# robot-learning-freiburg/MM-DistillNet

Measured on AMD Instinct MI355X. Metric: distillation-step images/sec (3 teachers + audio student, D2, bs=8), higher is better.
Workload: dtype f32; 1 GPU; BASELINE configs[2]: full 3-teacher (RGB+thermal+depth) -> audio student distillation step, EfficientDet-D2, 512x512, per-GPU batch 8, fwd+losses+bwd+all-reduce+Adam; global_batch=8, image_size=512, parallelism=dp1, graph=True, full=False

## Files before the change

mm_distillnet_amd/csrc/elt.hip:

```cpp
#include "common.h"
#include <cstdlib>

#define ROWS_PER_BLOCK 256
static inline int elt_rows_per_block(long long M, int C, bool reduces = false) {
  const long long blocks = (long long)cdiv(C, 64) * cdiv(M, ROWS_PER_BLOCK);
  int rpb = blocks >= 1024 ? ROWS_PER_BLOCK : (blocks >= 256 ? 128 : 64);
  while (reduces && rpb < ROWS_PER_BLOCK && cdiv(M, rpb) > 64) rpb *= 2;
  return rpb;
}

__device__ __forceinline__ float4 red_rowgroups(float4 v) {
  v.x += __shfl_xor(v.x, 16, 64); v.y += __shfl_xor(v.y, 16, 64); v.z += __shfl_xor(v.z, 16, 64); v.w += __shfl_xor(v.w, 16, 64);
  v.x += __shfl_xor(v.x, 32, 64); v.y += __shfl_xor(v.y, 32, 64); v.z += __shfl_xor(v.z, 32, 64); v.w += __shfl_xor(v.w, 32, 64);
  return v;
}
__device__ __forceinline__ float block_chan_sum(float4 v, float* sRed , int tid) {
  v = red_rowgroups(v);
  __syncthreads();
  if ((tid & 63) < 16) *reinterpret_cast<float4*>(&sRed[(tid >> 6) * 64 + (tid & 15) * 4]) = v;
  __syncthreads();
  float r = 0.f;
  if (tid < 64) r = sRed[tid] + sRed[64 + tid] + sRed[128 + tid] + sRed[192 + tid];
  return r;
}
// ... 248 lines not shown
  if (images_per_group <= 0 || w_stride <= 0 || bn_stride <= 0 || (w_stride & 3) || (bn_stride & 3)) return MMD_EINVAL;
  g_group = MmdGroup{n_groups, images_per_group, w_stride, bn_stride};
  g_group_read = false;
  return MMD_OK;
}

template <bool Q>
__global__ __launch_bounds__(256) void se_hidden_kernel(const void* __restrict__ pooled_, const float* __restrict__ wr,
                                                        const float* __restrict__ br, float* __restrict__ hpre, int C, int S,
                                                        int g_images, long long g_w) {
  const int b = blockIdx.x, wave = threadIdx.x >> 6, lane = threadIdx.x & 63;
  const int j = blockIdx.y * 4 + wave;
  if (j >= S) return;
  if (g_images) { const size_t o = (size_t)(b / g_images) * g_w; wr += o; br += o; }
  const float* p = reinterpret_cast<const float*>(pooled_) + (size_t)b * C;
  const long long* pq = reinterpret_cast<const long long*>(pooled_) + (size_t)b * C;
  const float* w = wr + (size_t)j * C;
  float acc = 0.f;
#pragma unroll 4
  for (int c = lane * 4; c < C; c += 256) {
    float4 a;
    if (Q) {
      const longlong2 q0 = *reinterpret_cast<const longlong2*>(pq + c), q1 = *reinterpret_cast<const longlong2*>(pq + c + 2);
      a = make_float4(mmd_pool_get(q0.x), mmd_pool_get(q0.y), mmd_pool_get(q1.x), mmd_pool_get(q1.y));
    } else {
      a = mmd_ld4(p + c);
    }
    const float4 q = mmd_ld4(w + c);
    acc += a.x * q.x + a.y * q.y + a.z * q.z + a.w * q.w;
  }
  acc = wave_sum(acc);
  if (lane == 0) hpre[(size_t)b * S + j] = acc + br[j];
}
__global__ __launch_bounds__(256) void se_gate_kernel(const float* __restrict__ hpre, const float* __restrict__ wet,
                                                      const float* __restrict__ be, float* __restrict__ gate, int C, int S,
                                                      int g_images, long long g_w) {
  __shared__ float sh[256];
  const int b = blockIdx.x;
  if (g_images) { const size_t o = (size_t)(b / g_images) * g_w; wet += o; be += o; }
  for (int j = threadIdx.x; j < S; j += 256) sh[j] = mmd_swish(hpre[(size_t)b * S + j]);
  __syncthreads();
  const int c = blockIdx.y * 256 + threadIdx.x;
  if (c >= C) return;
  float acc = be[c];
#pragma unroll 8
  for (int j = 0; j < S; ++j) acc += wet[(size_t)j * C + c] * sh[j];
  gate[(size_t)b * C + c] = mmd_sigmoid(acc);
}
static int se_fc_fwd_impl(const void* pooled, bool q, const float* wr, const float* br, const float* we, const float* be,
                          float* hpre, float* gate, int B, int C, int S, hipStream_t stream) {
  if (!pooled || !wr || !br || !we || !be || !hpre || !gate || B <= 0 || C <= 0 || (C & 3) || S <= 0 || S > 256) return MMD_EINVAL;
  const MmdGroup& gr = mmd_group();
  const int gi = gr.n > 1 ? gr.images : 0;
  if (gi && B != gr.n * gr.images) return MMD_EINVAL;
  mmd_prof_tag(MMD_FAM_SE, "sefwd B%lld C%lld S%lld q%lld", B, C, S, q ? 1 : 0);
  mmd_prof_begin(MMD_FAM_SE, stream);
  if (q) hipLaunchKernelGGL(se_hidden_kernel<true>, dim3(B, cdiv(S, 4)), dim3(256), 0, stream, pooled, wr, br, hpre, C, S, gi, gr.w_stride);
  else hipLaunchKernelGGL(se_hidden_kernel<false>, dim3(B, cdiv(S, 4)), dim3(256), 0, stream, pooled, wr, br, hpre, C, S, gi, gr.w_stride);
  hipLaunchKernelGGL(se_gate_kernel, dim3(B, cdiv(C, 256)), dim3(256), 0, stream, hpre, we, be, gate, C, S, gi, gr.w_stride);
  mmd_prof_end(MMD_FAM_SE, stream, 4.0 * B * (double)C * S, 4.0 * ((gr.n > 1 ? gr.n : 1) * 2.0 * C * S + (double)B * ((q ? 3.0 : 2.0) * C + 2.0 * S)));
  return mmd_check_launch();
}
extern "C" int mmd_se_fc_fwd(const float* pooled, const float* wr, const float* br, const float* we, const float* be,
                             float* hpre, float* gate, int B, int C, int S, hipStream_t stream) {
  return se_fc_fwd_impl(pooled, false, wr, br, we, be, hpre, gate, B, C, S, stream);
}
extern "C" int mmd_se_fc_fwd_q(const long long* pooled_q, const float* wr, const float* br, const float* we, const float* be,
                               float* hpre, float* gate, int B, int C, int S, hipStream_t stream) {
  return se_fc_fwd_impl(pooled_q, true, wr, br, we, be, hpre, gate, B, C, S, stream);
}

__global__ __launch_bounds__(256) void se_bwd_a_kernel(const float* __restrict__ dgate, const float* __restrict__ gate,
                                                       const float* __restrict__ wet, float* __restrict__ dpe, float* dh,
                                                       int C, int S) {
  const int b = blockIdx.x, wave = threadIdx.x >> 6, lane = threadIdx.x & 63;
  const int j = blockIdx.y * 4 + wave;
  if (j >= S) return;
  const float* gp = gate + (size_t)b * C;
  const float* dp = dgate + (size_t)b * C;
  const float* wp = wet + (size_t)j * C;
  float acc = 0.f;
#pragma unroll 4
  for (int c = lane * 4; c < C; c += 256) {
    const float4 g = mmd_ld4(gp + c), dg = mmd_ld4(dp + c), w = mmd_ld4(wp + c);
    const float4 d = make_float4(dg.x * g.x * (1.f - g.x), dg.y * g.y * (1.f - g.y), dg.z * g.z * (1.f - g.z), dg.w * g.w * (1.f - g.w));
    if (j == 0) mmd_st4(dpe + (size_t)b * C + c, d);
    acc += w.x * d.x + w.y * d.y + w.z * d.z + w.w * d.w;
  }
  acc = wave_sum(acc);
  if (lane == 0) dh[(size_t)b * S + j] = acc;
}
__global__ __launch_bounds__(256) void se_bwd_b_kernel(const float* __restrict__ dh, const float* __restrict__ hpre,
                                                       const float* __restrict__ wr, float* __restrict__ dpr,
                                                       float* __restrict__ dpooled, float dpool_scale, int C, int S,
                                                       const float* __restrict__ gate, const float* __restrict__ pool5,
                                                       double* bn_sums, int B) {
  __shared__ float sd[256];
  const int b = blockIdx.x, tid = threadIdx.x;
  for (int j = tid; j < S; j += 256) {
    float d = dh[(size_t)b * S + j] * mmd_swish_grad(hpre[(size_t)b * S + j]);
    sd[j] = d;
    if (blockIdx.y == 0) dpr[(size_t)b * S + j] = d;
  }
  __syncthreads();
  const int c = blockIdx.y * 256 + tid;
  if (c >= C) return;
  float acc = 0.f;
#pragma unroll 8
  for (int j = 0; j < S; ++j) acc += wr[(size_t)j * C + c] * sd[j];
  const float dp = acc * dpool_scale;
  dpooled[(size_t)b * C + c] = dp;
  if (bn_sums) {
    const size_t i = (size_t)b * C + c, n = (size_t)B * C;
    const float gt = gate[i];
    atomicAdd(&bn_sums[c], (double)(gt * pool5[n + i] + dp * pool5[3 * n + i]));
    atomicAdd(&bn_sums[C + c], (double)(gt * pool5[2 * n + i] + dp * pool5[4 * n + i]));
  }
}
__global__ void se_fc_wgrad_kernel(const float* __restrict__ dpe, const float* __restrict__ dpr,
                                   const float* __restrict__ hpre, const float* __restrict__ pooled, float* dwr, float* dbr,
                                   float* dwe, float* dbe, int B, int C, int S) {
  int i = blockIdx.x * blockDim.x + threadIdx.x;
  if (i >= C * S) return;
  {
    int j = i / C, c = i % C;
    float acc = 0.f, accb = 0.f;
    for (int b = 0; b < B; ++b) {
      float d = dpe[(size_t)b * C + c];
      acc += d * mmd_swish(hpre[(size_t)b * S + j]);
      accb += d;
    }
    dwe[i] += acc;
    if (j == 0) dbe[c] += accb;
  }
  {
    int j = i / C, c = i % C;
    float acc = 0.f, accb = 0.f;
    for (int b = 0; b < B; ++b) {
      float d = dpr[(size_t)b * S + j];
      acc += d * pooled[(size_t)b * C + c];
      accb += d;
    }
    dwr[i] += acc;
    if (c == 0) dbr[j] += accb;
  }
}
extern "C" int mmd_se_fc_bwd(const float* dgate, const float* gate, const float* hpre, const float* pooled,
                             const float* wr, const float* we, float* dpe_ws, float* dpr_ws, float* dh_zeroed,
                             float* dpooled, float dpool_scale, float* dwr, float* dbr, float* dwe, float* dbe, int B,
                             int C, int S, const float* pool5, double* bn_sums, hipStream_t stream) {
  if (!dgate || !gate || !hpre || !pooled || !wr || !we || !dpe_ws || !dpr_ws || !dh_zeroed || !dpooled) return MMD_EINVAL;
  if (dwr && (!dbr || !dwe || !dbe)) return MMD_EINVAL;
  if (B <= 0 || C <= 0 || (C & 3) || S <= 0 || S > 256 || ((pool5 == nullptr) != (bn_sums == nullptr))) return MMD_EINVAL;
  mmd_prof_tag(MMD_FAM_SE, "sebwd B%lld C%lld S%lld", B, C, S, 0);
  mmd_prof_begin(MMD_FAM_SE, stream);
  hipLaunchKernelGGL(se_bwd_a_kernel, dim3(B, cdiv(S, 4)), dim3(256), 0, stream, dgate, gate, we, dpe_ws, dh_zeroed, C, S);
  hipLaunchKernelGGL(se_bwd_b_kernel, dim3(B, cdiv(C, 256)), dim3(256), 0, stream, dh_zeroed, hpre, wr, dpr_ws, dpooled,
                     dpool_scale, C, S, gate, pool5, bn_sums, B);
  if (dwr)
    hipLaunchKernelGGL(se_fc_wgrad_kernel, dim3(cdiv((long long)C * S, 256)), dim3(256), 0, stream, dpe_ws, dpr_ws, hpre,
                       pooled, dwr, dbr, dwe, dbe, B, C, S);
  mmd_prof_end(MMD_FAM_SE, stream, 4.0 * B * (double)C * S, 4.0 * (2.0 * C * S + (double)B * (4.0 * C + 3.0 * S)));
  return mmd_check_launch();
}
#define SE_MAXC 3072
__global__ __launch_bounds__(256) void se_bwd_ab_kernel(const float* __restrict__ dgate, const float* __restrict__ gate,
                                                        const float* __restrict__ hpre, const float* __restrict__ wr,
                                                        const float* __restrict__ wet, float* __restrict__ dpe, float* __restrict__ dpr,
                                                        float* __restrict__ dpooled, float dpool_scale, int C, int S,
                                                        const float* __restrict__ pool5, double* bn_sums, int B) {
  __shared__ float sdpe[SE_MAXC];
  __shared__ float sd[256];
  const int b = blockIdx.x, tid = threadIdx.x, wave = tid >> 6, lane = tid & 63;
  for (int c = tid; c < C; c += 256) {
    const float g = gate[(size_t)b * C + c];
    const float d = dgate[(size_t)b * C + c] * g * (1.f - g);
    sdpe[c] = d;
    if (blockIdx.y == 0) dpe[(size_t)b * C + c] = d;
  }
  __syncthreads();
  for (int j = wave; j < S; j += 4) {
    const float* w = wet + (size_t)j * C;
    float acc = 0.f;
    for (int c = lane; c < C; c += 64) acc += w[c] * sdpe[c];
    acc = wave_sum(acc);
    if (lane == 0) {
      const float d = acc * mmd_swish_grad(hpre[(size_t)b * S + j]);
      sd[j] = d;
      if (blockIdx.y == 0) dpr[(size_t)b * S + j] = d;
    }
  }
  __syncthreads();
  const int c = blockIdx.y * 256 + tid;
  if (c >= C) return;
  float acc = 0.f;
#pragma unroll 8
  for (int j = 0; j < S; ++j) acc += wr[(size_t)j * C + c] * sd[j];
  const float dp = acc * dpool_scale;
  dpooled[(size_t)b * C + c] = dp;
  if (bn_sums) {
    const size_t i = (size_t)b * C + c, n = (size_t)B * C;
    const float gt = gate[i];
    atomicAdd(&bn_sums[c], (double)(gt * pool5[n + i] + dp * pool5[3 * n + i]));
    atomicAdd(&bn_sums[C + c], (double)(gt * pool5[2 * n + i] + dp * pool5[4 * n + i]));
  }
}
extern "C" int mmd_se_fc_bwd_fused(const float* dgate, const float* gate, const float* hpre, const float* wr, const float* we,
                                   float* dpe_ws, float* dpr_ws, float* dpooled, float dpool_scale, int B, int C, int S,
                                   const float* pool5, double* bn_sums, hipStream_t stream) {
  if (!dgate || !gate || !hpre || !wr || !we || !dpe_ws || !dpr_ws || !dpooled) return MMD_EINVAL;
  if (B <= 0 || C <= 0 || C > SE_MAXC || S <= 0 || S > 256 || ((pool5 == nullptr) != (bn_sums == nullptr))) return MMD_EINVAL;
  mmd_prof_tag(MMD_FAM_SE, "sebwdf B%lld C%lld S%lld", B, C, S, 0);
  mmd_prof_begin(MMD_FAM_SE, stream);
  hipLaunchKernelGGL(se_bwd_ab_kernel, dim3(B, cdiv(C, 256)), dim3(256), 0, stream, dgate, gate, hpre, wr, we, dpe_ws, dpr_ws, dpooled,
                     dpool_scale, C, S, pool5, bn_sums, B);
  mmd_prof_end(MMD_FAM_SE, stream, 4.0 * B * (double)C * S, 4.0 * (2.0 * C * S + (double)B * (4.0 * C + 3.0 * S)));
  return mmd_check_launch();
}

struct SeWgDesc { const float* dpe; const float* dpr; const float* hpre; const float* pooled; float* dwr; float* dbr; float* dwe; float* dbe;
                  long long C; long long S; };
__global__ void se_fc_wgrad_batched_kernel(const SeWgDesc* __restrict__ desc, int B) {
  const SeWgDesc d = desc[blockIdx.y];
  const int C = (int)d.C, S = (int)d.S;
  const int i = blockIdx.x * blockDim.x + threadIdx.x;
  if (i >= C * S) return;
  const int j = i / C, c = i % C;
  float a1 = 0.f, b1 = 0.f, a2 = 0.f, b2 = 0.f;
  for (int b = 0; b < B; ++b) {
    const float pe = mmd_ldg(d.dpe + (size_t)b * C + c), pr = mmd_ldg(d.dpr + (size_t)b * S + j);
    a1 += pe * mmd_swish(mmd_ldg(d.hpre + (size_t)b * S + j)); b1 += pe;
    a2 += pr * mmd_ldg(d.pooled + (size_t)b * C + c); b2 += pr;
  }
  mmd_stg(d.dwe + i, mmd_ldg(d.dwe + i) + a1);
  if (j == 0) mmd_stg(d.dbe + c, mmd_ldg(d.dbe + c) + b1);
  mmd_stg(d.dwr + i, mmd_ldg(d.dwr + i) + a2);
  if (c == 0) mmd_stg(d.dbr + j, mmd_ldg(d.dbr + j) + b2);
}
extern "C" int mmd_se_fc_wgrad_batched(const void* desc, int n, int max_cs, int B, hipStream_t stream) {
  if (!desc || n <= 0 || max_cs <= 0 || B <= 0) return MMD_EINVAL;
  hipLaunchKernelGGL(se_fc_wgrad_batched_kernel, dim3(cdiv(max_cs, 256), n), dim3(256), 0, stream, (const SeWgDesc*)desc, B);
  return mmd_check_launch();
}

extern "C" int mmd_se_fc_wgrad(const float* dpe, const float* dpr, const float* hpre, const float* pooled, float* dwr, float* dbr,
                               float* dwe, float* dbe, int B, int C, int S, hipStream_t stream) {
  if (!dpe || !dpr || !hpre || !pooled || !dwr || !dbr || !dwe || !dbe || B <= 0 || C <= 0 || S <= 0 || S > 256) return MMD_EINVAL;
  hipLaunchKernelGGL(se_fc_wgrad_kernel, dim3(cdiv((long long)C * S, 256)), dim3(256), 0, stream, dpe, dpr, hpre, pooled, dwr,
// ... 495 lines not shown
```

mm_distillnet_amd/csrc/mbconv_fused.hip:

```cpp
#include "common.h"
#include <cstdlib>

struct MbxArgs {
  const float* x; const float* w0; const float* sc0; const float* sh0;
  const float* wd; const float* sc1; const float* sh1;
  float* y; long long* pool; float pool_scale;
  int B, H, W, Cin, C, OH, OW, pad_t, pad_l, tiles_h, tiles_w, cchunks;
  int y16;
  int g_images; long long g_w, g_bn;
};

template <int K, int S> struct MbxCfg;
template <> struct MbxCfg<3, 1> { static constexpr int TH = 16, TW = 16, R = 4; };
template <> struct MbxCfg<5, 1> { static constexpr int TH = 16, TW = 16, R = 4; };
template <> struct MbxCfg<3, 2> { static constexpr int TH = 8, TW = 8, R = 1; };
template <> struct MbxCfg<5, 2> { static constexpr int TH = 8, TW = 8, R = 1; };

constexpr int MBX_CC = 48;
constexpr int MBX_LD = 20;
constexpr int MBX_NW = 4;
static_assert(MBX_NW == 4, "the pool epilogue adds four wave slots in a fixed order");

template <int CTRL> __device__ __forceinline__ float mbx_dpp(float v) {
  return __int_as_float(__builtin_amdgcn_update_dpp(0, __float_as_int(v), CTRL, 0xf, 0xf, false));
}

template <int NK, int K, int S>
__global__ __launch_bounds__(MBX_NW * 64) void mbx_kernel(MbxArgs a) {
  using Cf = MbxCfg<K, S>;
  constexpr int TH = Cf::TH, TW = Cf::TW, R = Cf::R, NW = MBX_NW;
  constexpr int IH = (TH - 1) * S + K, IW = (TW - 1) * S + K, P = IH * IW;
  constexpr int PT = (P + 15) / 16, TPW = (PT + NW - 1) / NW;
  constexpr int NT = NW * 64, NG = NT / 4, CC = MBX_CC, LD = MBX_LD;
  constexpr int SEG = (R - 1) * S + K, NSTRIP = TH * (TW / R);
  constexpr int W0S = 4 * NK + 4;
  extern __shared__ float smem[];
  float* const sE = smem;
  float* const sW = smem + PT * 16 * LD;
  float* const sPool = sW + K * K * CC;
  float* const sAff = sPool + NW * CC;
  float* const sW0 = sAff + 4 * CC;
  const int tid = threadIdx.x, lane = tid & 63, r = lane & 15, g = lane >> 4;
  const int wave = __builtin_amdgcn_readfirstlane(tid >> 6);
  int bid = mmd_xcd_swizzle(blockIdx.x, gridDim.x);
  const int cc = bid % a.cchunks; bid /= a.cchunks;
  const int tw = bid % a.tiles_w; bid /= a.tiles_w;
  const int th = bid % a.tiles_h; bid /= a.tiles_h;
  const int b = bid, c0 = cc * CC;
  if (a.g_images) {
    const size_t gw = (size_t)(b / a.g_images) * a.g_w, gb = (size_t)(b / a.g_images) * a.g_bn;
    a.w0 += gw; a.wd += gw; a.sc0 += gb; a.sh0 += gb; a.sc1 += gb; a.sh1 += gb;
  }
  const int oh0 = th * TH, ow0 = tw * TW, ih0 = oh0 * S - a.pad_t, iw0 = ow0 * S - a.pad_l;
  const int H = a.H, W = a.W, Cin = a.Cin;

  float bx[TPW][NK];
  bool in[TPW];
  {
    const float* xb = a.x + (size_t)b * H * W * Cin + g * NK;
#pragma unroll
    for (int t = 0; t < TPW; ++t) {
      const int p = (wave + t * NW) * 16 + r;
      const int pr = p / IW, pc = p - pr * IW;
      const int ih = ih0 + pr, iw = iw0 + pc;
      in[t] = p < P && ih >= 0 && ih < H && iw >= 0 && iw < W;
      const int ihc = min(max(ih, 0), H - 1), iwc = min(max(iw, 0), W - 1);
      const float* xp = xb + ((size_t)ihc * W + iwc) * Cin;
      if (NK % 4 == 0) {
#pragma unroll
        for (int j = 0; j < NK; j += 4) {
          const float4 v = mmd_ld4(xp + j);
          bx[t][j] = v.x; bx[t][j + 1] = v.y; bx[t][j + 2] = v.z; bx[t][j + 3] = v.w;
        }
      } else {
#pragma unroll
      for (int j = 0; j < NK; j += 2) {
        const float2 v = *reinterpret_cast<const float2*>(xp + j);
        bx[t][j] = v.x; bx[t][j + 1] = v.y;
      }
      }
    }
  }
  for (int i = tid; i < K * K * 12; i += NT) {
    const int tap = i / 12, q = (i % 12) * 4;
    *reinterpret_cast<float4*>(&sW[tap * CC + q]) = mmd_ld4(a.wd + (size_t)tap * a.C + c0 + q);
  }
  for (int i = tid; i < CC * NK; i += NT) {
    const int n = i / NK, k4 = i - n * NK;
    *reinterpret_cast<float4*>(&sW0[n * W0S + k4 * 4]) = mmd_ld4(a.w0 + (size_t)c0 * Cin + i * 4);
  }
  if (tid < CC) {
    sAff[tid] = a.sc0[c0 + tid]; sAff[CC + tid] = a.sh0[c0 + tid]; sAff[2 * CC + tid] = a.sc1[c0 + tid]; sAff[3 * CC + tid] = a.sh1[c0 + tid];
  }
  __syncthreads();

  constexpr unsigned SPERM = S == 1 ? 0x73261540u : 0x76452310u;
  const int qd = tid & 3, grp = ((tid >> 5) << 3) + (int)((SPERM >> (((tid >> 2) & 7) * 4)) & 7u), c4 = qd * 4;
#pragma unroll 1
  for (int ct = 0; ct < 3; ++ct) {
    {
      float aw[NK];
      const float* wp = sW0 + (ct * 16 + r) * W0S + g * NK;
#pragma unroll
      for (int j = 0; j < NK; j += 2) {
        const float2 v = *reinterpret_cast<const float2*>(wp + j);
        aw[j] = v.x; aw[j + 1] = v.y;
      }
      const float4 s0 = *reinterpret_cast<const float4*>(&sAff[ct * 16 + 4 * g]), h0 = *reinterpret_cast<const float4*>(&sAff[CC + ct * 16 + 4 * g]);
#pragma unroll
      for (int t = 0; t < TPW; ++t) {
        const int tile = wave + t * NW;
        if (tile >= PT) break;
        f32x4 acc = f32x4{0.f, 0.f, 0.f, 0.f};
#pragma unroll
        for (int j = 0; j < NK; ++j) acc = __builtin_amdgcn_mfma_f32_16x16x4f32(aw[j], bx[t][j], acc, 0, 0, 0);
        float4 v;
        v.x = mmd_swish(acc[0] * s0.x + h0.x); v.y = mmd_swish(acc[1] * s0.y + h0.y);
        v.z = mmd_swish(acc[2] * s0.z + h0.z); v.w = mmd_swish(acc[3] * s0.w + h0.w);
        if (!in[t]) v = make_float4(0.f, 0.f, 0.f, 0.f);
        *reinterpret_cast<float4*>(&sE[(tile * 16 + r) * LD + 4 * g]) = v;
      }
    }
    __syncthreads();

    float4 pl = make_float4(0.f, 0.f, 0.f, 0.f);
    {
      const int cb = c0 + ct * 16 + c4;
      const float4 osc = *reinterpret_cast<const float4*>(&sAff[2 * CC + ct * 16 + c4]), osh = *reinterpret_cast<const float4*>(&sAff[3 * CC + ct * 16 + c4]);
      const float* const sWc = sW + ct * 16 + c4;
      for (int s = grp; s < NSTRIP; s += NG) {
        const int orow = s / (TW / R), ocol0 = (s % (TW / R)) * R;
        float4 acc[R];
#pragma unroll
        for (int o = 0; o < R; ++o) acc[o] = make_float4(0.f, 0.f, 0.f, 0.f);
#pragma unroll(K == 3 ? 3 : 1)
        for (int i = 0; i < K; ++i) {
          float4 in4[SEG];
          const float* prow = &sE[((orow * S + i) * IW + ocol0 * S) * LD + c4];
#pragma unroll
          for (int q = 0; q < SEG; ++q) in4[q] = *reinterpret_cast<const float4*>(prow + q * LD);
#pragma unroll
          for (int j = 0; j < K; ++j) {
            const float4 wv = *reinterpret_cast<const float4*>(&sWc[(i * K + j) * CC]);
#pragma unroll
            for (int o = 0; o < R; ++o) {
              acc[o].x += in4[o * S + j].x * wv.x; acc[o].y += in4[o * S + j].y * wv.y;
              acc[o].z += in4[o * S + j].z * wv.z; acc[o].w += in4[o * S + j].w * wv.w;
            }
          }
        }
        const int oh = oh0 + orow;
#pragma unroll
        for (int o = 0; o < R; ++o) {
          const int ow = ow0 + ocol0 + o;
          if (oh < a.OH && ow < a.OW) {
            float4 t;
            t.x = mmd_swish(acc[o].x * osc.x + osh.x); t.y = mmd_swish(acc[o].y * osc.y + osh.y);
            t.z = mmd_swish(acc[o].z * osc.z + osh.z); t.w = mmd_swish(acc[o].w * osc.w + osh.w);
            pl.x += t.x; pl.y += t.y; pl.z += t.z; pl.w += t.w;
            mmd_stw4(a.y, (((size_t)b * a.OH + oh) * a.OW + ow) * a.C + cb, t, a.y16);
          }
        }
      }
    }
    if (a.pool) {
      pl.x += mbx_dpp<0x124>(pl.x); pl.y += mbx_dpp<0x124>(pl.y); pl.z += mbx_dpp<0x124>(pl.z); pl.w += mbx_dpp<0x124>(pl.w);
      pl.x += mbx_dpp<0x128>(pl.x); pl.y += mbx_dpp<0x128>(pl.y); pl.z += mbx_dpp<0x128>(pl.z); pl.w += mbx_dpp<0x128>(pl.w);
      pl.x += __shfl_xor(pl.x, 16, 64); pl.y += __shfl_xor(pl.y, 16, 64); pl.z += __shfl_xor(pl.z, 16, 64); pl.w += __shfl_xor(pl.w, 16, 64);
      pl.x += __shfl_xor(pl.x, 32, 64); pl.y += __shfl_xor(pl.y, 32, 64); pl.z += __shfl_xor(pl.z, 32, 64); pl.w += __shfl_xor(pl.w, 32, 64);
      if (lane < 4) *reinterpret_cast<float4*>(sPool + wave * CC + ct * 16 + c4) = pl;
    }
    __syncthreads();
  }
  if (a.pool && tid < CC)
    mmd_pool_add(&a.pool[(size_t)b * a.C + c0 + tid], ((sPool[tid] + sPool[CC + tid]) + sPool[2 * CC + tid]) + sPool[3 * CC + tid], a.pool_scale);
}

static int mbx_same_pad_lo(int n, int k, int s, int* out) {
  int o = (n + s - 1) / s;
  int extra = (o - 1) * s - n + k;
  if (extra < 0) extra = 0;
  *out = o;
  return extra / 2;
}

template <int NK, int K, int S>
static int mbx_launch(MbxArgs& a, hipStream_t st) {
  using Cf = MbxCfg<K, S>;
  a.tiles_h = cdiv(a.OH, Cf::TH); a.tiles_w = cdiv(a.OW, Cf::TW); a.cchunks = a.C / MBX_CC;
  const long long nb = (long long)a.B * a.tiles_h * a.tiles_w * a.cchunks;
  if (nb > 0x7fffffffLL) return MMD_EINVAL;
  constexpr int IH = (Cf::TH - 1) * S + K, IW = (Cf::TW - 1) * S + K;
  constexpr size_t lds = (size_t)((IH * IW + 15) / 16 * 16 * MBX_LD + K * K * MBX_CC + (4 + MBX_NW) * MBX_CC + MBX_CC * (4 * NK + 4)) * sizeof(float);
  static_assert(lds <= 64 * 1024, "tile does not fit the default dynamic LDS limit");
  hipLaunchKernelGGL((mbx_kernel<NK, K, S>), dim3((unsigned)nb), dim3(MBX_NW * 64), lds, st, a);
  return mmd_check_launch();
}

template <int NK>
static int mbx_launch_ks(MbxArgs& a, int k, int s, hipStream_t st) {
  if (k == 3 && s == 1) return mbx_launch<NK, 3, 1>(a, st);
  if (k == 3 && s == 2) return mbx_launch<NK, 3, 2>(a, st);
  if (k == 5 && s == 1) return mbx_launch<NK, 5, 1>(a, st);
  return mbx_launch<NK, 5, 2>(a, st);
}

extern "C" int mmd_mbconv_expand_dw_supported(int Cin, int Cmid, int k, int stride) {
  if ((k != 3 && k != 5) || (stride != 1 && stride != 2)) return 0;
  if (Cmid <= 0 || Cmid % MBX_CC) return 0;
  return Cin == 16 || Cin == 24 || Cin == 32 || Cin == 40 || Cin == 48 || Cin == 56;
}

static int mbx_impl(const float* x, const float* w_expand, const float* scale0, const float* shift0,
                    const float* w_dw, const float* scale1, const float* shift1, float* y, long long* pool,
                    int B, int H, int W, int Cin, int Cmid, int k, int stride, int y16, hipStream_t stream) {
  if (!x || !w_expand || !scale0 || !shift0 || !w_dw || !scale1 || !shift1 || !y || B <= 0 || H <= 0 || W <= 0) return MMD_EINVAL;
  if (!mmd_mbconv_expand_dw_supported(Cin, Cmid, k, stride)) return MMD_EINVAL;
  MbxArgs a{};
  a.x = x; a.w0 = w_expand; a.sc0 = scale0; a.sh0 = shift0; a.wd = w_dw; a.sc1 = scale1; a.sh1 = shift1; a.y = y; a.pool = pool;
  a.B = B; a.H = H; a.W = W; a.Cin = Cin; a.C = Cmid;
  a.pad_t = mbx_same_pad_lo(H, k, stride, &a.OH); a.pad_l = mbx_same_pad_lo(W, k, stride, &a.OW);
  a.pool_scale = 1.0f / (float)((long long)a.OH * a.OW);
  a.y16 = y16;
  if (mmd_group_on()) {
    const MmdGroup& gr = mmd_group();
    if (B != gr.n * gr.images || y16) return MMD_EINVAL;
    a.g_images = gr.images; a.g_w = gr.w_stride; a.g_bn = gr.bn_stride;
// ... 28 lines not shown
```

Measured before the change: 597.0 images/sec.

## Fuse SE forward FCs into one kernel and prefetch gate-weight columns

Adds a single-launch SE forward kernel that stages pooled activations in shared memory, computes the hidden FC with multi-row wave dot products, and then computes the gate FC in the same block. This removes a launch and the round trip of the hidden activations through global memory. The column dot products now prefetch the first 32 weight rows into registers before the barrier, and the fused backward kernel is reused for the unfused bwd path when no weight grads are needed. The cost is redundant hidden-FC work per C-tile block, which is limited by a byte threshold, plus higher register pressure.

```diff
diff --git a/mm_distillnet_amd/csrc/elt.hip b/mm_distillnet_amd/csrc/elt.hip
--- a/mm_distillnet_amd/csrc/elt.hip
+++ b/mm_distillnet_amd/csrc/elt.hip
@@ -304,20 +304,117 @@
   acc = wave_sum(acc);
   if (lane == 0) hpre[(size_t)b * S + j] = acc + br[j];
 }
+#define SE_GU 32
+struct SeCol { float v[SE_GU]; };
+__device__ __forceinline__ SeCol se_col_load(const float* __restrict__ w, int C, int c, int S, int j0) {
+  SeCol q;
+#pragma unroll
+  for (int u = 0; u < SE_GU; ++u) q.v[u] = w[(size_t)min(j0 + u, S - 1) * C + c];
+  return q;
+}
+__device__ __forceinline__ float se_col_add(float acc, const SeCol& q, const float* sh, int S, int j0) {
+  if (j0 + SE_GU <= S) {
+#pragma unroll
+    for (int u = 0; u < SE_GU; ++u) acc += q.v[u] * sh[j0 + u];
+  } else {
+#pragma unroll
+    for (int u = 0; u < SE_GU; ++u)
+      if (j0 + u < S) acc += q.v[u] * sh[j0 + u];
+  }
+  return acc;
+}
+__device__ __forceinline__ float se_col_dot(float acc, const SeCol& first, const float* __restrict__ w, int C, int c, int S, const float* sh) {
+  acc = se_col_add(acc, first, sh, S, 0);
+  for (int j0 = SE_GU; j0 < S; j0 += SE_GU) acc = se_col_add(acc, se_col_load(w, C, c, S, j0), sh, S, j0);
+  return acc;
+}
 __global__ __launch_bounds__(256) void se_gate_kernel(const float* __restrict__ hpre, const float* __restrict__ wet,
                                                       const float* __restrict__ be, float* __restrict__ gate, int C, int S,
                                                       int g_images, long long g_w) {
   __shared__ float sh[256];
   const int b = blockIdx.x;
   if (g_images) { const size_t o = (size_t)(b / g_images) * g_w; wet += o; be += o; }
+  const int c = blockIdx.y * 256 + threadIdx.x, cc = min(c, C - 1);
+  const SeCol first = se_col_load(wet, C, cc, S, 0);
+  const float bias = be[cc];
   for (int j = threadIdx.x; j < S; j += 256) sh[j] = mmd_swish(hpre[(size_t)b * S + j]);
   __syncthreads();
-  const int c = blockIdx.y * 256 + threadIdx.x;
   if (c >= C) return;
-  float acc = be[c];
-#pragma unroll 8
-  for (int j = 0; j < S; ++j) acc += wet[(size_t)j * C + c] * sh[j];
-  gate[(size_t)b * C + c] = mmd_sigmoid(acc);
+  gate[(size_t)b * C + c] = mmd_sigmoid(se_col_dot(bias, first, wet, C, c, S, sh));
+}
+#define SE_MAXC 3072
+#define SE_JU 8
+#ifndef SE_ONE_MAX_BYTES
+#define SE_ONE_MAX_BYTES (8ll << 20)
+#endif
+static inline bool se_one_launch(int B, int C, int S) {
+  return C <= SE_MAXC && 4ll * B * cdiv(C, 256) * S * C <= (long long)(SE_ONE_MAX_BYTES);
+}
+template <class Pre, class Emit>
+__device__ __forceinline__ void se_hidden_rows(const float* sv, const float* __restrict__ w, int C, int S, int wave, int lane, Pre pre, Emit emit) {
+  for (int j0 = wave; j0 < S; j0 += 4 * SE_JU) {
+    const float* wp[SE_JU];
+    float acc[SE_JU], pv[SE_JU];
+#pragma unroll
+    for (int u = 0; u < SE_JU; ++u) {
+      const int j = min(j0 + 4 * u, S - 1);
+      wp[u] = w + (size_t)j * C;
+      pv[u] = pre(j);
+      acc[u] = 0.f;
+    }
+#pragma unroll 2
+    for (int c = lane * 4; c < C; c += 256) {
+      float4 q[SE_JU];
+#pragma unroll
+      for (int u = 0; u < SE_JU; ++u) q[u] = mmd_ld4(wp[u] + c);
+      const float4 a = mmd_ld4(sv + c);
+#pragma unroll
+      for (int u = 0; u < SE_JU; ++u) acc[u] += a.x * q[u].x + a.y * q[u].y + a.z * q[u].z + a.w * q[u].w;
+    }
+#pragma unroll
+    for (int o = 32; o > 0; o >>= 1)
+#pragma unroll
+      for (int u = 0; u < SE_JU; ++u) acc[u] += __shfl_xor(acc[u], o, 64);
+    if (lane == 0)
+#pragma unroll
+      for (int u = 0; u < SE_JU; ++u)
+        if (j0 + 4 * u < S) emit(j0 + 4 * u, acc[u], pv[u]);
+  }
+}
+template <bool Q>
+__global__ __launch_bounds__(256) void se_fwd_kernel(const void* __restrict__ pooled_, const float* __restrict__ wr,
+                                                     const float* __restrict__ br, const float* __restrict__ wet,
+                                                     const float* __restrict__ be, float* __restrict__ hpre, float* __restrict__ gate,
+                                                     int C, int S, int g_images, long long g_w) {
+  __shared__ __attribute__((aligned(16))) float sp[SE_MAXC];
+  __shared__ float sh[256];
+  const int b = blockIdx.x, tid = threadIdx.x;
+  if (g_images) { const size_t o = (size_t)(b / g_images) * g_w; wr += o; br += o; wet += o; be += o; }
+  const int cg = blockIdx.y * 256 + tid, cgc = min(cg, C - 1);
+  const SeCol gfirst = se_col_load(wet, C, cgc, S, 0);
+  const float gbias = be[cgc];
+  for (int c = tid * 4; c < C; c += 1024) {
+    float4 a;
+    if (Q) {
+      const long long* pq = reinterpret_cast<const long long*>(pooled_) + (size_t)b * C + c;
+      const longlong2 q0 = *reinterpret_cast<const longlong2*>(pq), q1 = *reinterpret_cast<const longlong2*>(pq + 2);
+      a = make_float4(mmd_pool_get(q0.x), mmd_pool_get(q0.y), mmd_pool_get(q1.x), mmd_pool_get(q1.y));
+    } else {
+      a = mmd_ld4(reinterpret_cast<const float*>(pooled_) + (size_t)b * C + c);
+    }
+    mmd_st4(sp + c, a);
+  }
+  __syncthreads();
+  const bool first = blockIdx.y == 0;
+  se_hidden_rows(sp, wr, C, S, tid >> 6, tid & 63, [&](int j) { return br[j]; },
+                 [&](int j, float dot, float bias) {
+                   const float h = dot + bias;
+                   sh[j] = mmd_swish(h);
+                   if (first) hpre[(size_t)b * S + j] = h;
+                 });
+  __syncthreads();
+  if (cg >= C) return;
+  gate[(size_t)b * C + cg] = mmd_sigmoid(se_col_dot(gbias, gfirst, wet, C, cg, S, sh));
 }
 static int se_fc_fwd_impl(const void* pooled, bool q, const float* wr, const float* br, const float* we, const float* be,
                           float* hpre, float* gate, int B, int C, int S, hipStream_t stream) {
@@ -327,9 +424,14 @@
   if (gi && B != gr.n * gr.images) return MMD_EINVAL;
   mmd_prof_tag(MMD_FAM_SE, "sefwd B%lld C%lld S%lld q%lld", B, C, S, q ? 1 : 0);
   mmd_prof_begin(MMD_FAM_SE, stream);
-  if (q) hipLaunchKernelGGL(se_hidden_kernel<true>, dim3(B, cdiv(S, 4)), dim3(256), 0, stream, pooled, wr, br, hpre, C, S, gi, gr.w_stride);
-  else hipLaunchKernelGGL(se_hidden_kernel<false>, dim3(B, cdiv(S, 4)), dim3(256), 0, stream, pooled, wr, br, hpre, C, S, gi, gr.w_stride);
-  hipLaunchKernelGGL(se_gate_kernel, dim3(B, cdiv(C, 256)), dim3(256), 0, stream, hpre, we, be, gate, C, S, gi, gr.w_stride);
+  if (se_one_launch(B, C, S)) {
+    if (q) hipLaunchKernelGGL(se_fwd_kernel<true>, dim3(B, cdiv(C, 256)), dim3(256), 0, stream, pooled, wr, br, we, be, hpre, gate, C, S, gi, gr.w_stride);
+    else hipLaunchKernelGGL(se_fwd_kernel<false>, dim3(B, cdiv(C, 256)), dim3(256), 0, stream, pooled, wr, br, we, be, hpre, gate, C, S, gi, gr.w_stride);
+  } else {
+    if (q) hipLaunchKernelGGL(se_hidden_kernel<true>, dim3(B, cdiv(S, 4)), dim3(256), 0, stream, pooled, wr, br, hpre, C, S, gi, gr.w_stride);
+    else hipLaunchKernelGGL(se_hidden_kernel<false>, dim3(B, cdiv(S, 4)), dim3(256), 0, stream, pooled, wr, br, hpre, C, S, gi, gr.w_stride);
+    hipLaunchKernelGGL(se_gate_kernel, dim3(B, cdiv(C, 256)), dim3(256), 0, stream, hpre, we, be, gate, C, S, gi, gr.w_stride);
+  }
   mmd_prof_end(MMD_FAM_SE, stream, 4.0 * B * (double)C * S, 4.0 * ((gr.n > 1 ? gr.n : 1) * 2.0 * C * S + (double)B * ((q ? 3.0 : 2.0) * C + 2.0 * S)));
   return mmd_check_launch();
 }
@@ -369,18 +471,16 @@
                                                        double* bn_sums, int B) {
   __shared__ float sd[256];
   const int b = blockIdx.x, tid = threadIdx.x;
+  const int c = blockIdx.y * 256 + tid;
+  const SeCol first = se_col_load(wr, C, min(c, C - 1), S, 0);
   for (int j = tid; j < S; j += 256) {
     float d = dh[(size_t)b * S + j] * mmd_swish_grad(hpre[(size_t)b * S + j]);
     sd[j] = d;
     if (blockIdx.y == 0) dpr[(size_t)b * S + j] = d;
   }
   __syncthreads();
-  const int c = blockIdx.y * 256 + tid;
   if (c >= C) return;
-  float acc = 0.f;
-#pragma unroll 8
-  for (int j = 0; j < S; ++j) acc += wr[(size_t)j * C + c] * sd[j];
-  const float dp = acc * dpool_scale;
+  const float dp = se_col_dot(0.f, first, wr, C, c, S, sd) * dpool_scale;
   dpooled[(size_t)b * C + c] = dp;
   if (bn_sums) {
     const size_t i = (size_t)b * C + c, n = (size_t)B * C;
@@ -417,6 +517,9 @@
     if (c == 0) dbr[j] += accb;
   }
 }
+__global__ void se_bwd_ab_kernel(const float* dgate, const float* gate, const float* hpre, const float* wr, const float* wet, float* dpe,
+                                 float* dpr, float* dh, float* dpooled, float dpool_scale, int C, int S, const float* pool5,
+                                 double* bn_sums, int B);
 extern "C" int mmd_se_fc_bwd(const float* dgate, const float* gate, const float* hpre, const float* pooled,
                              const float* wr, const float* we, float* dpe_ws, float* dpr_ws, float* dh_zeroed,
                              float* dpooled, float dpool_scale, float* dwr, float* dbr, float* dwe, float* dbe, int B,
@@ -426,49 +529,51 @@
   if (B <= 0 || C <= 0 || (C & 3) || S <= 0 || S > 256 || ((pool5 == nullptr) != (bn_sums == nullptr))) return MMD_EINVAL;
   mmd_prof_tag(MMD_FAM_SE, "sebwd B%lld C%lld S%lld", B, C, S, 0);
   mmd_prof_begin(MMD_FAM_SE, stream);
-  hipLaunchKernelGGL(se_bwd_a_kernel, dim3(B, cdiv(S, 4)), dim3(256), 0, stream, dgate, gate, we, dpe_ws, dh_zeroed, C, S);
-  hipLaunchKernelGGL(se_bwd_b_kernel, dim3(B, cdiv(C, 256)), dim3(256), 0, stream, dh_zeroed, hpre, wr, dpr_ws, dpooled,
-                     dpool_scale, C, S, gate, pool5, bn_sums, B);
+  if (!dwr && se_one_launch(B, C, S)) {
+    hipLaunchKernelGGL(se_bwd_ab_kernel, dim3(B, cdiv(C, 256)), dim3(256), 0, stream, dgate, gate, hpre, wr, we, dpe_ws, dpr_ws, dh_zeroed,
+                       dpooled, dpool_scale, C, S, pool5, bn_sums, B);
+  } else {
+    hipLaunchKernelGGL(se_bwd_a_kernel, dim3(B, cdiv(S, 4)), dim3(256), 0, stream, dgate, gate, we, dpe_ws, dh_zeroed, C, S);
+    hipLaunchKernelGGL(se_bwd_b_kernel, dim3(B, cdiv(C, 256)), dim3(256), 0, stream, dh_zeroed, hpre, wr, dpr_ws, dpooled,
+                       dpool_scale, C, S, gate, pool5, bn_sums, B);
+  }
   if (dwr)
     hipLaunchKernelGGL(se_fc_wgrad_kernel, dim3(cdiv((long long)C * S, 256)), dim3(256), 0, stream, dpe_ws, dpr_ws, hpre,
                        pooled, dwr, dbr, dwe, dbe, B, C, S);
   mmd_prof_end(MMD_FAM_SE, stream, 4.0 * B * (double)C * S, 4.0 * (2.0 * C * S + (double)B * (4.0 * C + 3.0 * S)));
   return mmd_check_launch();
 }
-#define SE_MAXC 3072
 __global__ __launch_bounds__(256) void se_bwd_ab_kernel(const float* __restrict__ dgate, const float* __restrict__ gate,
                                                         const float* __restrict__ hpre, const float* __restrict__ wr,
                                                         const float* __restrict__ wet, float* __restrict__ dpe, float* __restrict__ dpr,
-                                                        float* __restrict__ dpooled, float dpool_scale, int C, int S,
+                                                        float* __restrict__ dh, float* __restrict__ dpooled, float dpool_scale, int C, int S,
                                                         const float* __restrict__ pool5, double* bn_sums, int B) {
-  __shared__ float sdpe[SE_MAXC];
+  __shared__ __attribute__((aligned(16))) float sdpe[SE_MAXC];
   __shared__ float sd[256];
-  const int b = blockIdx.x, tid = threadIdx.x, wave = tid >> 6, lane = tid & 63;
-  for (int c = tid; c < C; c += 256) {
-    const float g = gate[(size_t)b * C + c];
-    const float d = dgate[(size_t)b * C + c] * g * (1.f - g);
-    sdpe[c] = d;
-    if (blockIdx.y == 0) dpe[(size_t)b * C + c] = d;
+  const int b = blockIdx.x, tid = threadIdx.x;
+  const bool first = blockIdx.y == 0;
+  const int cp = blockIdx.y * 256 + tid;
+  const SeCol pfirst = se_col_load(wr, C, min(cp, C - 1), S, 0);
+  for (int c = tid * 4; c < C; c += 1024) {
+    const float4 g = mmd_ld4(gate + (size_t)b * C + c), dg = mmd_ld4(dgate + (size_t)b * C + c);
+    const float4 d = make_float4(dg.x * g.x * (1.f - g.x), dg.y * g.y * (1.f - g.y), dg.z * g.z * (1.f - g.z), dg.w * g.w * (1.f - g.w));
+    mmd_st4(sdpe + c, d);
+    if (first) mmd_st4(dpe + (size_t)b * C + c, d);
   }
   __syncthreads();
-  for (int j = wave; j < S; j += 4) {
-    const float* w = wet + (size_t)j * C;
-    float acc = 0.f;
-    for (int c = lane; c < C; c += 64) acc += w[c] * sdpe[c];
-    acc = wave_sum(acc);
-    if (lane == 0) {
-      const float d = acc * mmd_swish_grad(hpre[(size_t)b * S + j]);
-      sd[j] = d;
-      if (blockIdx.y == 0) dpr[(size_t)b * S + j] = d;
-    }
-  }
+  se_hidden_rows(sdpe, wet, C, S, tid >> 6, tid & 63, [&](int j) { return mmd_swish_grad(hpre[(size_t)b * S + j]); },
+                 [&](int j, float dot, float sg) {
+                   const float d = dot * sg;
+                   sd[j] = d;
+                   if (first) {
+                     dpr[(size_t)b * S + j] = d;
+                     if (dh) dh[(size_t)b * S + j] = dot;
+                   }
+                 });
   __syncthreads();
-  const int c = blockIdx.y * 256 + tid;
+  const int c = cp;
   if (c >= C) return;
-  float acc = 0.f;
-#pragma unroll 8
-  for (int j = 0; j < S; ++j) acc += wr[(size_t)j * C + c] * sd[j];
-  const float dp = acc * dpool_scale;
+  const float dp = se_col_dot(0.f, pfirst, wr, C, c, S, sd) * dpool_scale;
   dpooled[(size_t)b * C + c] = dp;
   if (bn_sums) {
     const size_t i = (size_t)b * C + c, n = (size_t)B * C;
@@ -481,11 +586,11 @@
                                    float* dpe_ws, float* dpr_ws, float* dpooled, float dpool_scale, int B, int C, int S,
                                    const float* pool5, double* bn_sums, hipStream_t stream) {
   if (!dgate || !gate || !hpre || !wr || !we || !dpe_ws || !dpr_ws || !dpooled) return MMD_EINVAL;
-  if (B <= 0 || C <= 0 || C > SE_MAXC || S <= 0 || S > 256 || ((pool5 == nullptr) != (bn_sums == nullptr))) return MMD_EINVAL;
+  if (B <= 0 || C <= 0 || C > SE_MAXC || (C & 3) || S <= 0 || S > 256 || ((pool5 == nullptr) != (bn_sums == nullptr))) return MMD_EINVAL;
   mmd_prof_tag(MMD_FAM_SE, "sebwdf B%lld C%lld S%lld", B, C, S, 0);
   mmd_prof_begin(MMD_FAM_SE, stream);
-  hipLaunchKernelGGL(se_bwd_ab_kernel, dim3(B, cdiv(C, 256)), dim3(256), 0, stream, dgate, gate, hpre, wr, we, dpe_ws, dpr_ws, dpooled,
-                     dpool_scale, C, S, pool5, bn_sums, B);
+  hipLaunchKernelGGL(se_bwd_ab_kernel, dim3(B, cdiv(C, 256)), dim3(256), 0, stream, dgate, gate, hpre, wr, we, dpe_ws, dpr_ws,
+                     (float*)nullptr, dpooled, dpool_scale, C, S, pool5, bn_sums, B);
   mmd_prof_end(MMD_FAM_SE, stream, 4.0 * B * (double)C * S, 4.0 * (2.0 * C * S + (double)B * (4.0 * C + 3.0 * S)));
   return mmd_check_launch();
 }
```

Result: no change. 602.3 images/sec (median of 6 runs) (+0.9%).

## Double-buffer expanded tile in LDS to overlap next expand MFMA with depthwise conv

Applied to the files above, without the earlier changes.

For stride-1 MBConv expand+depthwise kernels, the expanded activation tile is double-buffered in LDS. The next channel chunk's pointwise MFMA expansion is interleaved with the current chunk's depthwise rows (row-pipelined for k=3), which removes one barrier per chunk and hides MFMA latency behind LDS/VALU work. The strip loop is flattened to one strip per 4-lane group, and launch bounds now request two blocks per CU. In exchange, LDS use grows, possibly past 64KB (handled by raising the dynamic LDS attribute), and register pressure rises, which could reduce occupancy. Optional timestamp probes are added but compiled out by default.

```diff
diff --git a/mm_distillnet_amd/csrc/mbconv_fused.hip b/mm_distillnet_amd/csrc/mbconv_fused.hip
--- a/mm_distillnet_amd/csrc/mbconv_fused.hip
+++ b/mm_distillnet_amd/csrc/mbconv_fused.hip
@@ -10,33 +10,68 @@
   int g_images; long long g_w, g_bn;
 };
 
-template <int K, int S> struct MbxCfg;
-template <> struct MbxCfg<3, 1> { static constexpr int TH = 16, TW = 16, R = 4; };
-template <> struct MbxCfg<5, 1> { static constexpr int TH = 16, TW = 16, R = 4; };
-template <> struct MbxCfg<3, 2> { static constexpr int TH = 8, TW = 8, R = 1; };
-template <> struct MbxCfg<5, 2> { static constexpr int TH = 8, TW = 8, R = 1; };
-
 constexpr int MBX_CC = 48;
 constexpr int MBX_LD = 20;
 constexpr int MBX_NW = 4;
 static_assert(MBX_NW == 4, "the pool epilogue adds four wave slots in a fixed order");
 
+template <int K_, int S_, int TH_, int TW_, int R_, int NEB_> struct MbxTile {
+  static constexpr int K = K_, S = S_, TH = TH_, TW = TW_, R = R_;
+  static constexpr int IH = (TH - 1) * S + K, IW = (TW - 1) * S + K, P = IH * IW;
+  static constexpr int PT = (P + 15) / 16, TPW = (PT + MBX_NW - 1) / MBX_NW;
+  static constexpr int EBUF = PT * 16 * MBX_LD;
+  static constexpr int NEB = NEB_;
+  static constexpr int NSTRIP = TH * (TW / R);
+  static_assert(NSTRIP == MBX_NW * 16, "phase 2 deals exactly one strip to each 4-lane group");
+  static constexpr size_t lds(int nk) { return (size_t)(NEB * EBUF + K * K * MBX_CC + (4 + MBX_NW) * MBX_CC + MBX_CC * (4 * nk + 4)) * sizeof(float); }
+  static int tiles_h(int OH) { return cdiv(OH, TH); }
+  static int tiles_w(int OW) { return cdiv(OW, TW); }
+};
+template <int K, int S> struct MbxCfg;
+template <> struct MbxCfg<3, 1> : MbxTile<3, 1, 16, 16, 4, 2> {};
+template <> struct MbxCfg<5, 1> : MbxTile<5, 1, 16, 16, 4, 2> {};
+template <> struct MbxCfg<3, 2> : MbxTile<3, 2, 8, 8, 1, 1> {};
+template <> struct MbxCfg<5, 2> : MbxTile<5, 2, 8, 8, 1, 1> {};
+
 template <int CTRL> __device__ __forceinline__ float mbx_dpp(float v) {
   return __int_as_float(__builtin_amdgcn_update_dpp(0, __float_as_int(v), CTRL, 0xf, 0xf, false));
 }
 
+#ifdef MMD_MBXSTAMPS
+__device__ unsigned long long g_mbxst[16];
+#define MMD_XT(i) do { if (blockIdx.x == 0 && threadIdx.x == 0) g_mbxst[i] = wall_clock64(); } while (0)
+extern "C" int mmd_mbx_stamps(unsigned long long* out) { return hipMemcpyFromSymbol(out, HIP_SYMBOL(g_mbxst), sizeof(g_mbxst)) == hipSuccess ? 0 : -1; }
+#else
+#define MMD_XT(i)
+#endif
+
+template <int NK>
+__device__ __forceinline__ f32x4 mbx_expand_tile(const float (&aw)[NK], const float (&bx)[NK]) {
+  f32x4 acc = f32x4{0.f, 0.f, 0.f, 0.f};
+#pragma unroll
+  for (int j = 0; j < NK; ++j) acc = __builtin_amdgcn_mfma_f32_16x16x4f32(aw[j], bx[j], acc, 0, 0, 0);
+  return acc;
+}
+__device__ __forceinline__ void mbx_expand_store(float* dst, const f32x4& acc, const float4& s0, const float4& h0, bool in) {
+  float4 v;
+  v.x = mmd_swish(acc[0] * s0.x + h0.x); v.y = mmd_swish(acc[1] * s0.y + h0.y);
+  v.z = mmd_swish(acc[2] * s0.z + h0.z); v.w = mmd_swish(acc[3] * s0.w + h0.w);
+  if (!in) v = make_float4(0.f, 0.f, 0.f, 0.f);
+  *reinterpret_cast<float4*>(dst) = v;
+}
+
 template <int NK, int K, int S>
-__global__ __launch_bounds__(MBX_NW * 64) void mbx_kernel(MbxArgs a) {
+__global__ __launch_bounds__(MBX_NW * 64, 2) void mbx_kernel(MbxArgs a) {
   using Cf = MbxCfg<K, S>;
   constexpr int TH = Cf::TH, TW = Cf::TW, R = Cf::R, NW = MBX_NW;
-  constexpr int IH = (TH - 1) * S + K, IW = (TW - 1) * S + K, P = IH * IW;
-  constexpr int PT = (P + 15) / 16, TPW = (PT + NW - 1) / NW;
-  constexpr int NT = NW * 64, NG = NT / 4, CC = MBX_CC, LD = MBX_LD;
-  constexpr int SEG = (R - 1) * S + K, NSTRIP = TH * (TW / R);
+  constexpr int IW = Cf::IW, P = Cf::P, PT = Cf::PT, TPW = Cf::TPW, EBUF = Cf::EBUF;
+  constexpr int NT = NW * 64, CC = MBX_CC, LD = MBX_LD;
+  constexpr int SEG = (R - 1) * S + K;
+  constexpr bool PIPE = Cf::NEB == 2, ROWPIPE = PIPE && K == 3;
   constexpr int W0S = 4 * NK + 4;
   extern __shared__ float smem[];
   float* const sE = smem;
-  float* const sW = smem + PT * 16 * LD;
+  float* const sW = smem + Cf::NEB * EBUF;
   float* const sPool = sW + K * K * CC;
   float* const sAff = sPool + NW * CC;
   float* const sW0 = sAff + 4 * CC;
@@ -53,6 +88,7 @@
   }
   const int oh0 = th * TH, ow0 = tw * TW, ih0 = oh0 * S - a.pad_t, iw0 = ow0 * S - a.pad_l;
   const int H = a.H, W = a.W, Cin = a.Cin;
+  MMD_XT(0);
 
   float bx[TPW][NK];
   bool in[TPW];
@@ -93,74 +129,108 @@
     sAff[tid] = a.sc0[c0 + tid]; sAff[CC + tid] = a.sh0[c0 + tid]; sAff[2 * CC + tid] = a.sc1[c0 + tid]; sAff[3 * CC + tid] = a.sh1[c0 + tid];
   }
   __syncthreads();
+  MMD_XT(1);
 
   constexpr unsigned SPERM = S == 1 ? 0x73261540u : 0x76452310u;
   const int qd = tid & 3, grp = ((tid >> 5) << 3) + (int)((SPERM >> (((tid >> 2) & 7) * 4)) & 7u), c4 = qd * 4;
-#pragma unroll 1
+  const int orow = grp / (TW / R), ocol0 = (grp % (TW / R)) * R;
+  const int erow = (wave * 16 + r) * LD + 4 * g;
+
+  auto load_w0 = [&](int ct, float (&aw)[NK], float4& s0, float4& h0) {
+    const float* wp = sW0 + (ct * 16 + r) * W0S + g * NK;
+#pragma unroll
+    for (int j = 0; j < NK; j += 2) {
+      const float2 v = *reinterpret_cast<const float2*>(wp + j);
+      aw[j] = v.x; aw[j + 1] = v.y;
+    }
+    s0 = *reinterpret_cast<const float4*>(&sAff[ct * 16 + 4 * g]); h0 = *reinterpret_cast<const float4*>(&sAff[CC + ct * 16 + 4 * g]);
+  };
+  auto expand_all = [&](int ct, float* dst) {
+    float aw[NK]; float4 s0, h0;
+    load_w0(ct, aw, s0, h0);
+#pragma unroll
+    for (int t = 0; t < TPW; ++t) {
+      if ((t + 1) * NW > PT && wave + t * NW >= PT) break;
+      const f32x4 acc = mbx_expand_tile<NK>(aw, bx[t]);
+      mbx_expand_store(dst + erow + t * NW * 16 * LD, acc, s0, h0, in[t]);
+    }
+  };
+  if (PIPE) {
+    expand_all(0, sE);
+    MMD_XT(2);
+    __syncthreads();
+    MMD_XT(3);
+  }
+
+#pragma unroll
   for (int ct = 0; ct < 3; ++ct) {
-    {
-      float aw[NK];
-      const float* wp = sW0 + (ct * 16 + r) * W0S + g * NK;
-#pragma unroll
-      for (int j = 0; j < NK; j += 2) {
-        const float2 v = *reinterpret_cast<const float2*>(wp + j);
-        aw[j] = v.x; aw[j + 1] = v.y;
-      }
-      const float4 s0 = *reinterpret_cast<const float4*>(&sAff[ct * 16 + 4 * g]), h0 = *reinterpret_cast<const float4*>(&sAff[CC + ct * 16 + 4 * g]);
-#pragma unroll
-      for (int t = 0; t < TPW; ++t) {
-        const int tile = wave + t * NW;
-        if (tile >= PT) break;
-        f32x4 acc = f32x4{0.f, 0.f, 0.f, 0.f};
-#pragma unroll
-        for (int j = 0; j < NK; ++j) acc = __builtin_amdgcn_mfma_f32_16x16x4f32(aw[j], bx[t][j], acc, 0, 0, 0);
-        float4 v;
-        v.x = mmd_swish(acc[0] * s0.x + h0.x); v.y = mmd_swish(acc[1] * s0.y + h0.y);
-        v.z = mmd_swish(acc[2] * s0.z + h0.z); v.w = mmd_swish(acc[3] * s0.w + h0.w);
-        if (!in[t]) v = make_float4(0.f, 0.f, 0.f, 0.f);
-        *reinterpret_cast<float4*>(&sE[(tile * 16 + r) * LD + 4 * g]) = v;
-      }
-    }
-    __syncthreads();
-
+    if (!PIPE) {
+      expand_all(ct, sE);
+      __syncthreads();
+    }
+    const float* const sEc = sE + (PIPE ? (ct & 1) * EBUF : 0);
+    float* const sEn = sE + ((ct + 1) & 1) * EBUF + erow;
+    const bool more = PIPE && ct < 2;
+    float aw[NK]; float4 s0, h0;
+    if (more) load_w0(ct + 1, aw, s0, h0);
+    f32x4 eacc[TPW];
+
+    const float4 osc = *reinterpret_cast<const float4*>(&sAff[2 * CC + ct * 16 + c4]), osh = *reinterpret_cast<const float4*>(&sAff[3 * CC + ct * 16 + c4]);
+    const float* const sWc = sW + ct * 16 + c4;
+    float4 acc[R];
+#pragma unroll
+    for (int o = 0; o < R; ++o) acc[o] = make_float4(0.f, 0.f, 0.f, 0.f);
+    if (more && !ROWPIPE) {
+#pragma unroll
+      for (int t = 0; t < TPW; ++t)
+        if ((t + 1) * NW <= PT) eacc[t] = mbx_expand_tile<NK>(aw, bx[t]);
+    }
+#pragma unroll(ROWPIPE ? K : 1)
+    for (int i = 0; i < K; ++i) {
+      if (ROWPIPE && more) {
+#pragma unroll
+        for (int t = 0; t < TPW; ++t)
+          if (t * K / TPW == i && (t + 1) * NW <= PT) eacc[t] = mbx_expand_tile<NK>(aw, bx[t]);
+      }
+      float4 in4[SEG];
+      const float* prow = &sEc[((orow * S + i) * IW + ocol0 * S) * LD + c4];
+#pragma unroll
+      for (int q = 0; q < SEG; ++q) in4[q] = mmd_lds_ld4(prow + q * LD);
+      if (ROWPIPE && more && i > 0) {
+#pragma unroll
+        for (int t = 0; t < TPW; ++t)
+          if (t * K / TPW == i - 1 && (t + 1) * NW <= PT) mbx_expand_store(sEn + t * NW * 16 * LD, eacc[t], s0, h0, in[t]);
+      }
+#pragma unroll
+      for (int j = 0; j < K; ++j) {
+        const float4 wv = mmd_lds_ld4(&sWc[(i * K + j) * CC]);
+#pragma unroll
+        for (int o = 0; o < R; ++o) {
+          acc[o].x += in4[o * S + j].x * wv.x; acc[o].y += in4[o * S + j].y * wv.y;
+          acc[o].z += in4[o * S + j].z * wv.z; acc[o].w += in4[o * S + j].w * wv.w;
+        }
+      }
+    }
+    if (more) {
+#pragma unroll
+      for (int t = 0; t < TPW; ++t)
+        if ((!ROWPIPE || t * K / TPW == K - 1) && (t + 1) * NW <= PT) mbx_expand_store(sEn + t * NW * 16 * LD, eacc[t], s0, h0, in[t]);
+      if (TPW * NW > PT && wave + (TPW - 1) * NW < PT)
+        mbx_expand_store(sEn + (TPW - 1) * NW * 16 * LD, mbx_expand_tile<NK>(aw, bx[TPW - 1]), s0, h0, in[TPW - 1]);
+    }
     float4 pl = make_float4(0.f, 0.f, 0.f, 0.f);
     {
       const int cb = c0 + ct * 16 + c4;
-      const float4 osc = *reinterpret_cast<const float4*>(&sAff[2 * CC + ct * 16 + c4]), osh = *reinterpret_cast<const float4*>(&sAff[3 * CC + ct * 16 + c4]);
-      const float* const sWc = sW + ct * 16 + c4;
-      for (int s = grp; s < NSTRIP; s += NG) {
-        const int orow = s / (TW / R), ocol0 = (s % (TW / R)) * R;
-        float4 acc[R];
-#pragma unroll
-        for (int o = 0; o < R; ++o) acc[o] = make_float4(0.f, 0.f, 0.f, 0.f);
-#pragma unroll(K == 3 ? 3 : 1)
-        for (int i = 0; i < K; ++i) {
-          float4 in4[SEG];
-          const float* prow = &sE[((orow * S + i) * IW + ocol0 * S) * LD + c4];
-#pragma unroll
-          for (int q = 0; q < SEG; ++q) in4[q] = *reinterpret_cast<const float4*>(prow + q * LD);
-#pragma unroll
-          for (int j = 0; j < K; ++j) {
-            const float4 wv = *reinterpret_cast<const float4*>(&sWc[(i * K + j) * CC]);
-#pragma unroll
-            for (int o = 0; o < R; ++o) {
-              acc[o].x += in4[o * S + j].x * wv.x; acc[o].y += in4[o * S + j].y * wv.y;
-              acc[o].z += in4[o * S + j].z * wv.z; acc[o].w += in4[o * S + j].w * wv.w;
-            }
-          }
-        }
-        const int oh = oh0 + orow;
-#pragma unroll
-        for (int o = 0; o < R; ++o) {
-          const int ow = ow0 + ocol0 + o;
-          if (oh < a.OH && ow < a.OW) {
-            float4 t;
-            t.x = mmd_swish(acc[o].x * osc.x + osh.x); t.y = mmd_swish(acc[o].y * osc.y + osh.y);
-            t.z = mmd_swish(acc[o].z * osc.z + osh.z); t.w = mmd_swish(acc[o].w * osc.w + osh.w);
-            pl.x += t.x; pl.y += t.y; pl.z += t.z; pl.w += t.w;
-            mmd_stw4(a.y, (((size_t)b * a.OH + oh) * a.OW + ow) * a.C + cb, t, a.y16);
-          }
-        }
+      const int oh = oh0 + orow;
+#pragma unroll
+      for (int o = 0; o < R; ++o) {
+        const int ow = ow0 + ocol0 + o;
+        const bool ok = oh < a.OH && ow < a.OW;
+        float4 t;
+        t.x = mmd_swish(acc[o].x * osc.x + osh.x); t.y = mmd_swish(acc[o].y * osc.y + osh.y);
+        t.z = mmd_swish(acc[o].z * osc.z + osh.z); t.w = mmd_swish(acc[o].w * osc.w + osh.w);
+        pl.x += ok ? t.x : 0.f; pl.y += ok ? t.y : 0.f; pl.z += ok ? t.z : 0.f; pl.w += ok ? t.w : 0.f;
+        if (ok) mmd_stw4(a.y, (((size_t)b * a.OH + oh) * a.OW + ow) * a.C + cb, t, a.y16);
       }
     }
     if (a.pool) {
@@ -170,7 +240,9 @@
       pl.x += __shfl_xor(pl.x, 32, 64); pl.y += __shfl_xor(pl.y, 32, 64); pl.z += __shfl_xor(pl.z, 32, 64); pl.w += __shfl_xor(pl.w, 32, 64);
       if (lane < 4) *reinterpret_cast<float4*>(sPool + wave * CC + ct * 16 + c4) = pl;
     }
+    MMD_XT(4 + 2 * ct);
     __syncthreads();
+    MMD_XT(5 + 2 * ct);
   }
   if (a.pool && tid < CC)
     mmd_pool_add(&a.pool[(size_t)b * a.C + c0 + tid], ((sPool[tid] + sPool[CC + tid]) + sPool[2 * CC + tid]) + sPool[3 * CC + tid], a.pool_scale);
@@ -187,12 +259,18 @@
 template <int NK, int K, int S>
 static int mbx_launch(MbxArgs& a, hipStream_t st) {
   using Cf = MbxCfg<K, S>;
-  a.tiles_h = cdiv(a.OH, Cf::TH); a.tiles_w = cdiv(a.OW, Cf::TW); a.cchunks = a.C / MBX_CC;
+  a.tiles_h = Cf::tiles_h(a.OH); a.tiles_w = Cf::tiles_w(a.OW); a.cchunks = a.C / MBX_CC;
   const long long nb = (long long)a.B * a.tiles_h * a.tiles_w * a.cchunks;
   if (nb > 0x7fffffffLL) return MMD_EINVAL;
-  constexpr int IH = (Cf::TH - 1) * S + K, IW = (Cf::TW - 1) * S + K;
-  constexpr size_t lds = (size_t)((IH * IW + 15) / 16 * 16 * MBX_LD + K * K * MBX_CC + (4 + MBX_NW) * MBX_CC + MBX_CC * (4 * NK + 4)) * sizeof(float);
-  static_assert(lds <= 64 * 1024, "tile does not fit the default dynamic LDS limit");
+  constexpr size_t lds = Cf::lds(NK);
+  static_assert(2 * lds <= 160 * 1024, "two blocks must fit a CU's LDS: one block's barrier waits run beside the other's work");
+  if (lds > 64 * 1024) {
+    static bool attr = false;
+    if (!attr) {
+      if (hipFuncSetAttribute((const void*)mbx_kernel<NK, K, S>, hipFuncAttributeMaxDynamicSharedMemorySize, (int)lds) != hipSuccess) return MMD_ELAUNCH;
+      attr = true;
+    }
+  }
   hipLaunchKernelGGL((mbx_kernel<NK, K, S>), dim3((unsigned)nb), dim3(MBX_NW * 64), lds, st, a);
   return mmd_check_launch();
 }
```

Result: no change. 601.6 images/sec before, 597.0 images/sec after (-0.8%).
